# gonewest818/raytrace-clj

Hardware: NVIDIA B200
Metric: samples_per_sec (higher is better)
Workload: dtype f32

## Files before the change

### raytrace_clj_b200/csrc/rt_api.cu

```cuda
#include "../../include/raytrace_b200.h"

#include <cuda_runtime.h>
#include <dlfcn.h>
#include <math_constants.h>
#include <nccl.h>

#include <algorithm>
#include <cmath>
#include <cstdio>
#include <cstdlib>
#include <cstring>
#include <atomic>
#include <mutex>
#include <thread>
#include <string>
#include <vector>

#include "rt_bvh_build.cuh"
#include "rt_kernels.cuh"

using namespace rt;

namespace {

constexpr int kR = 4;
constexpr int kBlock = 256;
constexpr int kMinBlocks = 1;
constexpr int kTileCap = 4096;

thread_local std::string g_create_error;

struct DeviceBuffers {
    int dev = 0;
    cudaStream_t stream = nullptr;
    cudaEvent_t ev0 = nullptr, ev1 = nullptr, ev_done = nullptr;
    void* scene_blob = nullptr;
    void* scene_stage = nullptr;
    size_t scene_bytes = 0;
    DevScene sc{};
    float* d_sum = nullptr;
    float* d_mean = nullptr;
    uint8_t* d_rgb8 = nullptr;
    size_t frame_px = 0;
    unsigned long long* d_counters = nullptr;
    struct WaveLane {
        float4* queue = nullptr;
        unsigned long long* best = nullptr;
        uint2* pairs = nullptr;
        uint2* cands = nullptr;
        double* cand_t = nullptr;
        unsigned* cand_count = nullptr;
        WaveState* state = nullptr;
        LaneStatus* h_status = nullptr;
        LaneStatus* d_status = nullptr;
        cudaEvent_t ev_done = nullptr;
        cudaStream_t stream = nullptr;
        cudaStream_t stage_stream = nullptr;
        cudaEvent_t ev_culled = nullptr, ev_shaded = nullptr;
        size_t entries = 0;
        bool best_clean = false;
    } lanes[kMaxLanes];
    cudaEvent_t ev_lane_start = nullptr;
    TraceRec* d_trace = nullptr;
    struct TraceMeta { const char* kernel; int lane, iter; };
    std::vector<TraceMeta> trace_meta;
    void* scratch = nullptr;
    size_t scratch_bytes = 0;
    int sm_count = 0, clock_khz = 0;
    char name[64] = {0};
    float last_ms = 0.f;
    bool timed = false;
    float4* bvh_nodes = nullptr;
    size_t bvh_cap = 0;
    int bvh_builder = 0, bvh_depth = 0;
    long long bvh_build_ns = 0;
    void* bvh_scratch = nullptr;
    size_t bvh_scratch_bytes = 0;
    int* h_bvh_depth = nullptr;
    cudaEvent_t ev_b0 = nullptr, ev_b1 = nullptr;
    void* h_stage = nullptr;
    size_t h_stage_bytes = 0;
    cudaEvent_t ev_r0 = nullptr, ev_r1 = nullptr;
    cudaEvent_t ev_chunk[4] = {};
};

struct NcclApi {
    void* handle = nullptr;
    ncclResult_t (*CommInitAll)(ncclComm_t*, int, const int*) = nullptr;
    ncclResult_t (*CommDestroy)(ncclComm_t) = nullptr;
    ncclResult_t (*Reduce)(const void*, void*, size_t, ncclDataType_t, ncclRedOp_t, int, ncclComm_t, cudaStream_t) = nullptr;
    ncclResult_t (*GroupStart)() = nullptr;
    ncclResult_t (*GroupEnd)() = nullptr;
    const char* (*GetErrorString)(ncclResult_t) = nullptr;
    std::vector<ncclComm_t> comms;
};

}

struct Options {
    int wave_lanes = 2;
    long long wave_capacity = 1ll << 24;
    int cull_claims = 2;
    int cull_ctas_per_sm = 4;
    int cull_shape = 0;
    int light_block = 128;
    long long tail_entries = 1 << 19;
    int tail_ctas_per_sm = 0;
    int tile_records = 1024;
    int direct_spheres = 1;
    int common_origin = 1;
    int reduce = 0;
    int rows = 0;
    int tail_block = 256;
    int tail_rays = 1;
    int tail_solo = 24;
    int tail_lpp = 32;
    int mega_regcap = 0;
    int wave_depth = 2;
    int cull_tc = 1;
    int tc_tiles_per_cta = 0;
    int tc_ctas = 0;
    int bvh_build = 1;
};

struct rt_ctx {
    std::mutex mu;
    std::string err;
    std::vector<DeviceBuffers> devs;
    Options opt;
    bool has_scene = false, has_cam = false;
    int n_spheres = 0;
    int n_total = 0;
    int n_list = 0, n_cull = 0;
    int cull_cap = 0, preloaded = 0;
    int tc_tiles = 0;
    std::vector<std::vector<float>> tc_scratch_rows;
    std::vector<int> tc_row_k;
    int generic = 0;
    int accel = RT_ACCEL_BRUTE_FORCE;
    bool bvh_dirty = true;
    double win_lo = 0.0, win_hi = 0.0;
    std::vector<float> h_c0r, h_c1, h_t0t1;
    std::vector<unsigned> h_flags;
    std::vector<double> h_bs_c0, h_bs_c1, h_bs_r;
    DevCamera cam{};
    std::atomic<uint64_t> n_launches{0};
    std::mutex err_mu;
    bool profile = false;
    double stage_ms[4] = {0, 0, 0, 0};
    double reduce_ms = 0.0;
    std::vector<bool> peer_ok;
    NcclApi nccl;
};

namespace {

int fail(rt_ctx* ctx, int code, const std::string& msg) {
    if (ctx) {
        std::lock_guard<std::mutex> lk(ctx->err_mu);
        ctx->err = msg;
    } else {
        g_create_error = msg;
    }
    return code;
}

#define RT_CUDA(ctx, expr)                                                                          \
    do {                                                                                            \
        cudaError_t e__ = (expr);                                                                   \
        if (e__ != cudaSuccess)                                                                     \
            return fail(ctx, RT_ERR_CUDA, std::string(#expr) + ": " + cudaGetErrorString(e__));     \
    } while (0)

int ensure_scratch(rt_ctx* ctx, DeviceBuffers& d, size_t bytes) {
    if (d.scratch_bytes >= bytes) return RT_OK;
    if (d.scratch) cudaFree(d.scratch);
    d.scratch = nullptr;
    d.scratch_bytes = 0;
    RT_CUDA(ctx, cudaMalloc(&d.scratch, bytes));
    d.scratch_bytes = bytes;
    return RT_OK;
}

int ensure_frame(rt_ctx* ctx, DeviceBuffers& d, size_t px) {
    if (d.frame_px >= px) return RT_OK;
    if (d.d_sum) cudaFree(d.d_sum);
    if (d.d_mean) cudaFree(d.d_mean);
    if (d.d_rgb8) cudaFree(d.d_rgb8);
    d.d_sum = d.d_mean = nullptr;
    d.d_rgb8 = nullptr;
    d.frame_px = 0;
    RT_CUDA(ctx, cudaMalloc(&d.d_sum, px * 3 * sizeof(float)));
    RT_CUDA(ctx, cudaMalloc(&d.d_mean, px * 3 * sizeof(float)));
    RT_CUDA(ctx, cudaMalloc(&d.d_rgb8, px * 3));
    d.frame_px = px;
    return RT_OK;
}


void free_lane(DeviceBuffers::WaveLane& L) {
    if (L.queue) cudaFree(L.queue);
    if (L.best) cudaFree(L.best);
    if (L.pairs) cudaFree(L.pairs);
    if (L.cands) cudaFree(L.cands);
    if (L.cand_t) cudaFree(L.cand_t);
    if (L.cand_count) cudaFree(L.cand_count);
    L.queue = nullptr; L.best = nullptr; L.pairs = nullptr; L.cands = nullptr; L.cand_t = nullptr; L.cand_count = nullptr;
    L.entries = 0;
}

void free_wave(DeviceBuffers& d) {
    for (auto& L : d.lanes) {
        free_lane(L);
        if (L.state) cudaFree(L.state);
        if (L.h_status) cudaFreeHost(L.h_status);
        if (L.ev_done) cudaEventDestroy(L.ev_done);
        if (L.stream) cudaStreamDestroy(L.stream);
        if (L.stage_stream) cudaStreamDestroy(L.stage_stream);
        if (L.ev_culled) cudaEventDestroy(L.ev_culled);
        if (L.ev_shaded) cudaEventDestroy(L.ev_shaded);
        L = DeviceBuffers::WaveLane();
    }
    if (d.ev_lane_start) cudaEventDestroy(d.ev_lane_start);
    d.ev_lane_start = nullptr;
    if (d.d_trace) cudaFree(d.d_trace);
    d.d_trace = nullptr;
}

int ensure_lane(rt_ctx* ctx, DeviceBuffers& d, int lane, size_t entries) {
    DeviceBuffers::WaveLane& L = d.lanes[lane];
    if (!L.state) {
        RT_CUDA(ctx, cudaMalloc(&L.state, sizeof(WaveState)));
        RT_CUDA(ctx, cudaHostAlloc(&L.h_status, sizeof(LaneStatus), cudaHostAllocMapped));
        RT_CUDA(ctx, cudaHostGetDevicePointer((void**)&L.d_status, L.h_status, 0));
        RT_CUDA(ctx, cudaEventCreateWithFlags(&L.ev_done, cudaEventDisableTiming));
        if (lane > 0) RT_CUDA(ctx, cudaStreamCreateWithFlags(&L.stream, cudaStreamNonBlocking));
        int prio_least = 0, prio_greatest = 0;
        RT_CUDA(ctx, cudaDeviceGetStreamPriorityRange(&prio_least, &prio_greatest));
        RT_CUDA(ctx, cudaStreamCreateWithPriority(&L.stage_stream, cudaStreamNonBlocking, prio_greatest));
        RT_CUDA(ctx, cudaEventCreateWithFlags(&L.ev_culled, cudaEventDisableTiming));
        RT_CUDA(ctx, cudaEventCreateWithFlags(&L.ev_shaded, cudaEventDisableTiming));
        if (!d.ev_lane_start) RT_CUDA(ctx, cudaEventCreateWithFlags(&d.ev_lane_start, cudaEventDisableTiming));
    }
    if (L.entries >= entries) return RT_OK;
    free_lane(L);
    RT_CUDA(ctx, cudaMalloc(&L.queue, entries * 2 * 3 * sizeof(float4)));
    RT_CUDA(ctx, cudaMalloc(&L.best, entries * 2 * sizeof(unsigned long long)));
    RT_CUDA(ctx, cudaMalloc(&L.pairs, entries * kPairsPerEntry * sizeof(uint2)));
    const size_t cand_slots = entries * kPairsPerEntry + (size_t)d.sm_count * 8 * 8 * 32;
    RT_CUDA(ctx, cudaMalloc(&L.cands, cand_slots * sizeof(uint2)));
    RT_CUDA(ctx, cudaMalloc(&L.cand_t, cand_slots * sizeof(double)));
    RT_CUDA(ctx, cudaMalloc(&L.cand_count, (size_t)d.sm_count * 8 * 8 * sizeof(unsigned)));
    L.entries = entries;
    L.best_clean = false;
    return RT_OK;
}

size_t align_up(size_t x, size_t a) { return (x + a - 1) / a * a; }

float round_up_f32(double x) {
    float f = (float)x;
    if ((double)f < x) f = nextafterf(f, INFINITY);
    return f;
}

size_t mega_smem_bytes(int cull_cap) { return (size_t)cull_cap * sizeof(float4) + Culler<kR, kBlock>::LIST_BYTES; }

template <typename Kern>
int configure_kernel(rt_ctx* ctx, Kern kern, size_t smem, int* blocks_per_sm) {
    RT_CUDA(ctx, cudaFuncSetAttribute(kern, cudaFuncAttributeMaxDynamicSharedMemorySize, (int)smem));
    int b = 0;
    RT_CUDA(ctx, cudaOccupancyMaxActiveBlocksPerMultiprocessor(&b, kern, kBlock, smem));
    if (b < 1) return fail(ctx, RT_ERR_CUDA, "kernel does not fit on an SM");
    *blocks_per_sm = b;
    return RT_OK;
}

long long env_ll(const char* name, long long dflt) {
    const char* v = getenv(name);
    return (v && *v) ? atoll(v) : dflt;
}
int env_int(const char* name, int dflt) { return (int)env_ll(name, dflt); }

Options options_from_env() {
    Options o;
    o.wave_lanes = env_int("RT_WAVE_LANES", o.wave_lanes);
    o.wave_capacity = env_ll("RT_WAVE_CAPACITY", o.wave_capacity);
    o.cull_claims = env_int("RT_CULL_CLAIMS", o.cull_claims);
    o.cull_ctas_per_sm = env_int("RT_CULL_CTAS_PER_SM", o.cull_ctas_per_sm);
    const char* shape = getenv("RT_CULL_SHAPE");
    if (shape && !strcmp(shape, "128x6")) o.cull_shape = 1;
    if (shape && !strcmp(shape, "256x2")) o.cull_shape = 2;
    o.light_block = env_int("RT_LIGHT_BLOCK", o.light_block);
    o.tail_entries = env_ll("RT_TAIL_ENTRIES", o.tail_entries);
    o.tail_ctas_per_sm = env_int("RT_TAIL_CTAS_PER_SM", o.tail_ctas_per_sm);
    o.tile_records = env_int("RT_TILE_RECORDS", o.tile_records);
    o.direct_spheres = env_int("RT_DIRECT_SPHERES", o.direct_spheres);
    o.common_origin = env_int("RT_COMMON_ORIGIN", o.common_origin);
    o.reduce = env_int("RT_REDUCE", o.reduce);
    o.rows = env_int("RT_ROWS", o.rows);
    o.wave_depth = env_int("RT_WAVE_DEPTH", o.wave_depth);
    o.tail_rays = env_int("RT_TAIL_RAYS", o.tail_rays);
    o.tail_solo = env_int("RT_TAIL_SOLO", o.tail_solo);
    o.tail_lpp = env_int("RT_TAIL_LPP", o.tail_lpp);
    o.tail_block = env_int("RT_TAIL_BLOCK", o.tail_block);
    o.cull_tc = env_int("RT_CULL_TC", o.cull_tc);
    o.tc_tiles_per_cta = env_int("RT_TC_TILES_PER_CTA", o.tc_tiles_per_cta);
    o.tc_ctas = env_int("RT_TC_CTAS", o.tc_ctas);
    o.bvh_build = env_int("RT_BVH_BUILD", o.bvh_build);
    return o;
}

template <int BLOCK, int MINB>
int cull_config(rt_ctx* ctx, size_t* smem, int* bps, void (**kern)(const WaveParams)) {
    *kern = wf_cull<kR, BLOCK, MINB>;
    *smem = (ctx->preloaded ? 2 : 1) * (size_t)ctx->cull_cap * sizeof(float4) + Culler<kR, BLOCK>::LIST_BYTES;
    RT_CUDA(ctx, cudaFuncSetAttribute(*kern, cudaFuncAttributeMaxDynamicSharedMemorySize, (int)*smem));
    RT_CUDA(ctx, cudaOccupancyMaxActiveBlocksPerMultiprocessor(bps, *kern, BLOCK, *smem));
    if (*bps < 1) return fail(ctx, RT_ERR_CUDA, "cull kernel does not fit on an SM");
    return RT_OK;
}

int launch_wave(rt_ctx* ctx, DeviceBuffers& d, const RenderParams& P, unsigned long long, cudaStream_t stream) {
    const Options& opt = ctx->opt;
    void (*cull)(const WaveParams) = nullptr;
    size_t smem = 0;
    int bps = 0, cull_block = 256, rc;
    if (opt.cull_shape == 2) rc = cull_config<256, 2>(ctx, &smem, &bps, &cull);
    else if (opt.cull_shape == 1) { rc = cull_config<128, 6>(ctx, &smem, &bps, &cull); cull_block = 128; }
    else { rc = cull_config<128, 5>(ctx, &smem, &bps, &cull); cull_block = 128; }
    if (rc) return rc;
    const int cull_ctas_env = opt.cull_ctas_per_sm;
    if (cull_ctas_env > 0) bps = std::min(bps, cull_ctas_env);
    const size_t cap_env = (size_t)std::max<long long>(64, opt.wave_capacity);
    const int lanes_env = std::max(1, std::min(kMaxLanes, opt.wave_lanes));
    const int n_lanes = (ctx->profile || P.total_work < 65536) ? 1 : lanes_env;
    const size_t capacity = align_up((size_t)std::min<unsigned long long>(cap_env / n_lanes, (P.total_work + n_lanes - 1) / n_lanes), 32);

    bool done[kMaxLanes] = {};
    const unsigned tail_entries = (unsigned)std::max<long long>(0, opt.tail_entries);
    const bool gen = ctx->generic != 0;
    const bool tail4 = opt.tail_rays == 4;
    const int tail_block = (gen || tail4) ? 256 : (opt.tail_block == 32 || opt.tail_block == 64 || opt.tail_block == 128 ? opt.tail_block : 256);
    const size_t tail_smem = (size_t)ctx->cull_cap * sizeof(float4) +
                             (tail4 ? Culler<4, 256>::LIST_BYTES : (size_t)Culler<1, 256>::LIST_WORDS * tail_block * sizeof(uint32_t));
    int tail_bps = 0;
    void (*k_tail)(const WaveParams) = gen ? wf_tail<256, true, 1> : (tail4 ? wf_tail<256, false, 4> : wf_tail<256, false, 1>);
    if (tail_block == 128) k_tail = wf_tail<128, false, 1>;
    if (tail_block == 64) k_tail = wf_tail<64, false, 1>;
    if (tail_block == 32) k_tail = wf_tail<32, false, 1>;
    void (*k_refine)(const WaveParams) = gen ? wf_refine<true> : wf_refine<false>;
    void (*k_shade)(const WaveParams) = gen ? wf_shade<true> : wf_shade<false>;
    RT_CUDA(ctx, cudaFuncSetAttribute(k_tail, cudaFuncAttributeMaxDynamicSharedMemorySize, (int)tail_smem));
    RT_CUDA(ctx, cudaOccupancyMaxActiveBlocksPerMultiprocessor(&tail_bps, k_tail, tail_block, tail_smem));
    const int tail_auto = (n_lanes > 1 ? 1 : std::max(1, std::min((int)(tail_bps * tail_block / 256), 2))) * (256 / tail_block);
    const int tail_grid = d.sm_count * (opt.tail_ctas_per_sm > 0 ? opt.tail_ctas_per_sm : tail_auto);
    const bool bvh = ctx->accel == RT_ACCEL_BVH;
    void (*k_bvh)(const WaveParams) = gen ? wf_bvh<true> : wf_bvh<false>;
    const bool tail_ok = tail_bps >= 1 && tail_entries > 0 && !ctx->profile && !bvh;
    const bool use_tc = opt.cull_tc != 0 && ctx->tc_tiles > 0 && !bvh && ((ctx->n_list >= tc::MIN_LEAVES && !ctx->generic) || opt.cull_tc == 3);
    const int tc_launch_tiles = std::min(ctx->tc_tiles, (int)tc::MAX_TILES);
    const int tc_slots = tc::slots_for(tc_launch_tiles, 227 * 1024);
    const size_t tc_smem = tc::smem_bytes(tc_launch_tiles, tc_slots);
    if (use_tc) RT_CUDA(ctx, cudaFuncSetAttribute(wf_cull_tc, cudaFuncAttributeMaxDynamicSharedMemorySize, (int)tc_smem));
    const int tc_per_cta = std::max(0, opt.tc_tiles_per_cta);
    const int tc_grid = opt.tc_ctas > 0 ? std::min(opt.tc_ctas, 4 * d.sm_count) : d.sm_count;
    auto launch_tc = [&](const WaveParams& Wl, int per_cta, unsigned ctas, cudaStream_t s_) {
        WaveParams Wt = Wl;
        Wt.claims_per_warp = per_cta;
        Wt.tc_slots = tc_slots;
        for (int t0 = 0, pass = 0; t0 < ctx->tc_tiles; t0 += tc::MAX_TILES, ++pass) {
            Wt.tc_tile0 = t0;
            Wt.tc_launch_tiles = std::min((int)tc::MAX_TILES, ctx->tc_tiles - t0);
            Wt.tc_pass = pass;
            wf_cull_tc<<<ctas, tc::THREADS, tc_smem, s_>>>(Wt);
            if (pass) ctx->n_launches += 1;
        }
    };

    const int light_block = std::max(64, std::min(256, opt.light_block / 32 * 32));
    const int light_grid = d.sm_count * 8 * 256 / light_block;
    const int cull_grid = d.sm_count * bps;
    const int claims_env = std::max(0, opt.cull_claims);
    const int claims = (ctx->profile || !ctx->preloaded || n_lanes < 2 || bvh) ? 0 : claims_env;
    const int cull_warps = cull_block / 32, resident_warps = cull_grid * cull_warps;
    unsigned n_bound[kMaxLanes];
    WaveParams W[kMaxLanes];
    cudaStream_t st[kMaxLanes];
    unsigned long long first = 0;
    for (int l = 0; l < n_lanes; ++l) {
        if ((rc = ensure_lane(ctx, d, l, capacity))) return rc;
        DeviceBuffers::WaveLane& L = d.lanes[l];
        W[l] = WaveParams{};
        W[l].base = P;
        W[l].queue[0] = L.queue;
        W[l].queue[1] = L.queue + 3 * capacity;
        W[l].best_t = L.best;
        W[l].best_key = L.best + L.entries;
        W[l].pairs = L.pairs;
        W[l].cands = L.cands;
        W[l].cand_t = L.cand_t;
        W[l].cand_count = L.cand_count;
        W[l].st = L.state;
        W[l].capacity = (int)capacity;
        W[l].pair_cap = (unsigned)std::min<size_t>(capacity * kPairsPerEntry, 0xfffffff0u);
        W[l].cur = 0;
        W[l].claims_per_warp = claims;
        W[l].resident_warps = claims ? resident_warps : 0;
        W[l].tail_solo = (unsigned)std::max(0, opt.tail_solo);
        W[l].tail_lpp = opt.tail_lpp == 8 ? 8u : (opt.tail_lpp == 16 ? 16u : 32u);
        st[l] = l == 0 ? stream : L.stream;
    }
    static const char* trace_path = getenv("RT_TRACE");
    constexpr int kTraceMax = 8192;
    const bool tracing = trace_path && *trace_path;
    if (tracing) {
        if (!d.d_trace) RT_CUDA(ctx, cudaMalloc(&d.d_trace, kTraceMax * sizeof(TraceRec)));
        static const std::vector<TraceRec> init((size_t)kTraceMax, TraceRec{~0ull, 0ull});
        RT_CUDA(ctx, cudaMemcpyAsync(d.d_trace, init.data(), init.size() * sizeof(TraceRec), cudaMemcpyHostToDevice, stream));
        d.trace_meta.clear();
    }
    auto trace_slot = [&](const char* kernel, int lane, int iter) -> TraceRec* {
        if (!tracing || (int)d.trace_meta.size() >= kTraceMax) return nullptr;
        d.trace_meta.push_back({kernel, lane, iter});
        return d.d_trace + (d.trace_meta.size() - 1);
    };
    int iter_no[kMaxLanes] = {};
    static const bool debug_sync = getenv("RT_DEBUG_SYNC") && *getenv("RT_DEBUG_SYNC") == '1';
    auto dbg = [&](const char* what, int lane, int it) -> int {
        if (!debug_sync) return RT_OK;
        cudaError_t e = cudaDeviceSynchronize();
        if (e != cudaSuccess) return fail(ctx, RT_ERR_CUDA, std::string(what) + " (lane " + std::to_string(lane) + ", iteration " + std::to_string(it) + "): " + cudaGetErrorString(e));
        return RT_OK;
    };
    unsigned count0[kMaxLanes];
    unsigned long long total0 = 0;
    for (int l = 0; l < n_lanes; ++l) {
        count0[l] = (unsigned)std::min<unsigned long long>(capacity, P.total_work - total0);
        total0 += count0[l];
        n_bound[l] = count0[l];
    }
    InitParams I{};
    I.n_lanes = n_lanes;
    I.work_counter = P.work_counter;
    I.counters = P.counters;
    I.total0 = total0;
    I.total_work = P.total_work;
    for (int l = 0; l < n_lanes; ++l) {
        DeviceBuffers::WaveLane& L = d.lanes[l];
        I.st[l] = L.state;
        I.first[l] = first;
        I.count[l] = count0[l];
        first += count0[l];
        if (!L.best_clean) {
            wf_fill_best<<<d.sm_count * 4, 256, 0, stream>>>(L.best, L.best + L.entries, L.entries);
            ctx->n_launches += 1;
        }
        L.best_clean = false;
    }
    wf_init<<<1, 1, 0, stream>>>(I);
    ctx->n_launches += 1;
    RT_CUDA(ctx, cudaGetLastError());
    RT_CUDA(ctx, cudaEventRecord(d.ev_lane_start, stream));
    for (int l = 1; l < n_lanes; ++l) RT_CUDA(ctx, cudaStreamWaitEvent(st[l], d.ev_lane_start, 0));

    const int depth = std::max(1, std::min(16, opt.wave_depth));
    int enq[kMaxLanes] = {}, seen[kMaxLanes] = {};
    bool tailed[kMaxLanes] = {};
    for (int l = 0; l < n_lanes; ++l) {
        DeviceBuffers::WaveLane& L = d.lanes[l];
        memset(L.h_status, 0, sizeof(LaneStatus));
        W[l].status = L.d_status;
        if (count0[l] == 0) done[l] = true;
    }
    std::vector<cudaEvent_t> evs;
    unsigned idle_spins = 0;
    for (;;) {
        bool progressed = false, all_done = true;
        for (int l = 0; l < n_lanes; ++l) {
            if (done[l]) continue;
            all_done = false;
            DeviceBuffers::WaveLane& L = d.lanes[l];
            while (!tailed[l] && enq[l] - seen[l] < depth) {
                cudaEvent_t e[5] = {nullptr, nullptr, nullptr, nullptr, nullptr};
                if (ctx->profile)
                    for (auto& x : e) { RT_CUDA(ctx, cudaEventCreate(&x)); evs.push_back(x); }
                if (ctx->profile) cudaEventRecord(e[0], st[l]);
                W[l].iter = (unsigned)(enq[l] + 1);
                const bool tc_now = use_tc && !(enq[l] == 0 && P.common_origin && opt.cull_tc == 2);
                if (bvh) {
                    W[l].trace = trace_slot("bvh", l, iter_no[l]);
                    k_bvh<<<light_grid, 128, 0, st[l]>>>(W[l]);
                    if (ctx->profile) { cudaEventRecord(e[1], st[l]); cudaEventRecord(e[2], st[l]); cudaEventRecord(e[3], st[l]); }
                    W[l].trace = trace_slot("shade", l, iter_no[l]);
                    k_shade<<<light_grid, light_block, 0, st[l]>>>(W[l]);
                    if (ctx->profile) cudaEventRecord(e[4], st[l]);
                    ctx->n_launches -= 2;
                } else if (claims) {
                    W[l].trace = trace_slot("cull", l, iter_no[l]);
                    if (debug_sync) {
                        WaveState hs{};
                        cudaMemcpy(&hs, W[l].st, sizeof hs, cudaMemcpyDeviceToHost);
                        fprintf(stderr, "lane %d iteration %d cur %d: in flight %u fresh %u | other queue %u %u | mode %u exhausted %u npairs %u\n", l, enq[l], W[l].cur,
                                hs.cnt[W[l].cur][0], hs.cnt[W[l].cur][1], hs.cnt[W[l].cur ^ 1][0], hs.cnt[W[l].cur ^ 1][1], hs.mode, hs.exhausted, hs.npairs);
                    }
                    if (tc_now) {
                        const unsigned tiles = (n_bound[l] + tc::TILE_M - 1) / tc::TILE_M;
                        const unsigned ctas = tc_per_cta ? (tiles + (unsigned)tc_per_cta - 1u) / (unsigned)tc_per_cta : (unsigned)tc_grid;
                        launch_tc(W[l], tc_per_cta, std::max(1u, ctas), st[l]);
// ... 11 lines not shown
                    W[l].trace = trace_slot("tiebreak", l, iter_no[l]);
                    wf_tiebreak<<<light_grid, light_block, 0, L.stage_stream>>>(W[l]);
                    if ((rc = dbg("wf_tiebreak", l, enq[l]))) return rc;
                    W[l].trace = trace_slot("shade", l, iter_no[l]);
                    k_shade<<<light_grid, light_block, 0, L.stage_stream>>>(W[l]);
                    if ((rc = dbg("wf_shade", l, enq[l]))) return rc;
                    RT_CUDA(ctx, cudaEventRecord(L.ev_shaded, L.stage_stream));
                    RT_CUDA(ctx, cudaStreamWaitEvent(st[l], L.ev_shaded, 0));
                } else {
                    W[l].trace = trace_slot("cull", l, iter_no[l]);
                    if (tc_now) {
                        launch_tc(W[l], 0, (unsigned)tc_grid, st[l]);
                    } else {
                        cull<<<cull_grid, cull_block, smem, st[l]>>>(W[l]);
                    }
                    if (ctx->profile) cudaEventRecord(e[1], st[l]);
                    W[l].trace = trace_slot("refine", l, iter_no[l]);
                    k_refine<<<light_grid, light_block, 0, st[l]>>>(W[l]);
                    if (ctx->profile) cudaEventRecord(e[2], st[l]);
                    W[l].trace = trace_slot("tiebreak", l, iter_no[l]);
                    wf_tiebreak<<<light_grid, light_block, 0, st[l]>>>(W[l]);
                    if (ctx->profile) cudaEventRecord(e[3], st[l]);
                    W[l].trace = trace_slot("shade", l, iter_no[l]);
                    k_shade<<<light_grid, light_block, 0, st[l]>>>(W[l]);
                    if (ctx->profile) cudaEventRecord(e[4], st[l]);
                }
                RT_CUDA(ctx, cudaGetLastError());
                W[l].cur ^= 1;
                ++iter_no[l];
                ctx->n_launches += 4;
                ++enq[l];
                progressed = true;
            }
        }
        if (all_done) break;
        for (int l = 0; l < n_lanes; ++l) {
            if (done[l]) continue;
            DeviceBuffers::WaveLane& L = d.lanes[l];
            const volatile LaneStatus* hs = L.h_status;
            const unsigned seq = hs->seq;
            if ((int)seq == seen[l] && hs->mode != MODE_DONE) continue;
            std::atomic_thread_fence(std::memory_order_acquire);
            const unsigned n_next = hs->n_next, n_fresh = hs->n_fresh, exhausted = hs->exhausted, mode = hs->mode;
            if (hs->seq != seq) continue;
            seen[l] = (int)seq;
            progressed = true;
            if (exhausted) n_bound[l] = std::min(n_bound[l], n_next);
            if (mode == MODE_DONE) { done[l] = true; continue; }
            if (tail_ok && !tailed[l] && exhausted && n_fresh == 0 && n_next <= tail_entries) {
                W[l].iter = (unsigned)(enq[l] + 1);
                W[l].trace = trace_slot("tail", l, iter_no[l]);
                k_tail<<<tail_grid, tail_block, tail_smem, st[l]>>>(W[l]);
                if ((rc = dbg("wf_tail", l, enq[l]))) return rc;
                RT_CUDA(ctx, cudaGetLastError());
                ctx->n_launches += 1;
                tailed[l] = true;
            }
        }
        if (!progressed) {
            if (++idle_spins > 200) {
                if (cudaSuccess != cudaPeekAtLastError()) RT_CUDA(ctx, cudaGetLastError());
                if (idle_spins > 20000 && (idle_spins % 1000) == 0) {
                    for (int l = 0; l < n_lanes; ++l)
                        if (!done[l] && cudaStreamQuery(st[l]) == cudaSuccess && d.lanes[l].h_status->seq == (unsigned)seen[l] &&
                            enq[l] > seen[l])
                            return fail(ctx, RT_ERR_CUDA, "wavefront lane finished its queue without reporting status");
                }
                std::this_thread::yield();
            }
        } else {
            idle_spins = 0;
        }
    }
    for (int l = 1; l < n_lanes; ++l) {
        RT_CUDA(ctx, cudaEventRecord(d.lanes[l].ev_done, st[l]));
        RT_CUDA(ctx, cudaStreamWaitEvent(stream, d.lanes[l].ev_done, 0));
    }
    for (int l = 0; l < n_lanes; ++l) d.lanes[l].best_clean = true;
    if (ctx->profile) {
        RT_CUDA(ctx, cudaStreamSynchronize(stream));
        for (size_t i = 0; i + 4 < evs.size(); i += 5)
            for (int sgi = 0; sgi < 4; ++sgi) {
                float ms = 0.f;
                if (cudaEventElapsedTime(&ms, evs[i + sgi], evs[i + sgi + 1]) == cudaSuccess) ctx->stage_ms[sgi] += ms;
            }
        for (auto x : evs) cudaEventDestroy(x);
    }
    return RT_OK;
}

int launch_params(rt_ctx* ctx, DeviceBuffers& d, RenderParams& P, int variant, cudaStream_t stream);

int launch_render(rt_ctx* ctx, DeviceBuffers& d, int nx, int ny, int sample_begin, int sample_count, int row_offset,
                  int row_stride, int max_depth, uint64_t seed, int variant, float* d_sum, cudaStream_t stream) {
    RenderParams P{};
    P.sc = d.sc;
    P.cam = ctx->cam;
    P.nx = nx;
    P.ny = ny;
    P.sample_begin = sample_begin;
    P.sample_count = sample_count;
    P.row_offset = row_offset;
    P.row_stride = row_stride;
    P.rows_in_shard = (ny - row_offset + row_stride - 1) / row_stride;
    P.max_depth = max_depth;
    P.key = make_uint2((uint32_t)seed, (uint32_t)(seed >> 32));
    P.sum = d_sum;
    P.counters = d.d_counters;
// ... 873 lines not shown
    if (accel != RT_ACCEL_BRUTE_FORCE && accel != RT_ACCEL_BVH) return fail(ctx, RT_ERR_ARG, "unknown accelerator");
    ctx->accel = accel;
    if (accel == RT_ACCEL_BVH && ctx->has_scene) return ensure_bvh(ctx);
    return RT_OK;
}

int rt_get_bvh(rt_ctx* ctx, int device_index, float* out_nodes, int64_t cap_nodes, int64_t info[4]) {
    if (!ctx) return RT_ERR_ARG;
    std::lock_guard<std::mutex> lk(ctx->mu);
    if (int rc = check_ready(ctx)) return rc;
    if (device_index < 0 || device_index >= (int)ctx->devs.size()) return fail(ctx, RT_ERR_ARG, "device_index out of range");
    if (int rc = ensure_bvh(ctx)) return rc;
    DeviceBuffers& d = ctx->devs[(size_t)device_index];
    const int64_t n_nodes = d.sc.bvh_nodes;
    if (info) {
        info[0] = n_nodes;
        info[1] = d.bvh_depth;
        info[2] = d.bvh_builder;
        info[3] = d.bvh_build_ns;
    }
    if (out_nodes) {
        if (cap_nodes < n_nodes) return fail(ctx, RT_ERR_ARG, "cap_nodes is below the node count (info[0])");
        RT_CUDA(ctx, cudaSetDevice(d.dev));
        RT_CUDA(ctx, cudaMemcpy(out_nodes, d.bvh_nodes, (size_t)n_nodes * 4 * sizeof(float4), cudaMemcpyDeviceToHost));
        cudaSetDevice(ctx->devs[0].dev);
    }
    return RT_OK;
}

int rt_set_option(rt_ctx* ctx, const char* name, int64_t value) {
    if (!ctx) return RT_ERR_ARG;
    std::lock_guard<std::mutex> lk(ctx->mu);
    if (!name) return fail(ctx, RT_ERR_ARG, "option name is null");
    Options& o = ctx->opt;
    const std::string k(name);
    if (k == "wave_lanes") o.wave_lanes = (int)value;
    else if (k == "wave_capacity") o.wave_capacity = value;
    else if (k == "cull_claims") o.cull_claims = (int)value;
    else if (k == "cull_ctas_per_sm") o.cull_ctas_per_sm = (int)value;
    else if (k == "cull_shape") o.cull_shape = (int)value;
    else if (k == "light_block") o.light_block = (int)value;
    else if (k == "tail_entries") o.tail_entries = value;
    else if (k == "tail_ctas_per_sm") o.tail_ctas_per_sm = (int)value;
    else if (k == "tile_records") o.tile_records = (int)value;
    else if (k == "direct_spheres") o.direct_spheres = (int)value;
    else if (k == "common_origin") o.common_origin = (int)value;
    else if (k == "reduce") o.reduce = (int)value;
    else if (k == "rows") o.rows = (int)value;
    else if (k == "wave_depth") o.wave_depth = (int)value;
    else if (k == "mega_regcap") o.mega_regcap = (int)value;
    else if (k == "tail_rays") o.tail_rays = (int)value;
    else if (k == "tail_solo") o.tail_solo = (int)value;
    else if (k == "tail_lpp") o.tail_lpp = (int)value;
    else if (k == "tail_block") o.tail_block = (int)value;
    else if (k == "cull_tc") o.cull_tc = (int)value;
    else if (k == "tc_tiles_per_cta") o.tc_tiles_per_cta = (int)value;
    else if (k == "tc_ctas") o.tc_ctas = (int)value;
    else if (k == "bvh_build") o.bvh_build = (int)value;
    else return fail(ctx, RT_ERR_ARG, "unknown option: " + k);
    return RT_OK;
}

int rt_set_camera(rt_ctx* ctx, int cam_type, const float cam[24]) {
    if (!ctx) return RT_ERR_ARG;
    std::lock_guard<std::mutex> lk(ctx->mu);
    if (!cam) return fail(ctx, RT_ERR_ARG, "cam is null");
    if (cam_type != RT_CAM_PINHOLE && cam_type != RT_CAM_THIN_LENS) return fail(ctx, RT_ERR_UNSUPPORTED, "unknown camera type");
    DevCamera& c = ctx->cam;
    c.type = cam_type;
    auto g = [&](int k) { return make_float3(cam[3 * k], cam[3 * k + 1], cam[3 * k + 2]); };
    c.origin = g(0); c.lleft = g(1); c.horiz = g(2); c.vert = g(3); c.u = g(4); c.v = g(5); c.w = g(6);
    c.lens_radius = cam[21] / 2.0f;
    c.t0 = cam[22];
    c.t1 = cam[23];
    ctx->has_cam = true;
    return RT_OK;
}

int rt_render_accumulate_device(rt_ctx* ctx, int nx, int ny, int sample_begin, int sample_count, int row_offset,
                                int row_stride, int max_depth, uint64_t seed, int variant, float* d_sum, void* stream,
                                int sync) {
    int rc = check_ready(ctx);
    if (rc) return rc;
    std::lock_guard<std::mutex> lk(ctx->mu);
    if ((rc = check_camera_times(ctx))) return rc;
    if (nx <= 0 || ny <= 0 || sample_count < 0 || sample_begin < 0 || max_depth < 0 || !d_sum || row_stride < 1 ||
        row_offset < 0 || row_offset >= row_stride)
        return fail(ctx, RT_ERR_ARG, "bad render arguments");
    if ((long long)nx * ny > 0x7fffffffLL / 3) return fail(ctx, RT_ERR_ARG, "image too large");
    DeviceBuffers& d = ctx->devs[0];
    RT_CUDA(ctx, cudaSetDevice(d.dev));
    cudaStream_t st = (cudaStream_t)stream;
    RT_CUDA(ctx, cudaEventRecord(d.ev0, st));
    rc = launch_render(ctx, d, nx, ny, sample_begin, sample_count, row_offset, row_stride, max_depth, seed, variant, d_sum, st);
    if (rc) return rc;
    RT_CUDA(ctx, cudaEventRecord(d.ev1, st));
    d.timed = true;
    if (sync) RT_CUDA(ctx, cudaStreamSynchronize(st));
    return RT_OK;
}

int rt_resolve_device(rt_ctx* ctx, int nx, int ny, int nsamples_total, const float* d_sum, uint8_t* d_rgb8, void* stream,
                      int sync) {
    if (!ctx) return RT_ERR_ARG;
    std::lock_guard<std::mutex> lk(ctx->mu);
    if (nx <= 0 || ny <= 0 || nsamples_total <= 0 || !d_sum || !d_rgb8) return fail(ctx, RT_ERR_ARG, "bad resolve arguments");
// ... 584 lines not shown
```

### raytrace_clj_b200/csrc/rt_kernels.cuh

```cuda
#pragma once

#include "rt_device.cuh"

namespace rt {

#define RT_FOR_R _Pragma("unroll") for (int r = 0; r < R; ++r)

struct PathBounce {
    float o[3];
    float time;
    float d[3];
    int hit_id;
    double t;
};

struct RenderParams {
    DevScene sc;
    DevCamera cam;
    int nx, ny;
    int sample_begin, sample_count;
    int row_offset, row_stride, rows_in_shard;
    int max_depth;
    uint2 key;
    float* sum;
// ... 302 lines not shown
struct LaneStatus {
    unsigned n_next;
    unsigned n_fresh;
    unsigned exhausted;
    unsigned mode;
    unsigned seq;
    unsigned pad[3];
};
__device__ __forceinline__ unsigned wf_entry(unsigned i, unsigned n_g, unsigned n_p, unsigned capacity) {
    return i < n_g ? i : capacity - n_p + (i - n_g);
}

struct TraceRec {
    unsigned long long t_start, t_end;
};
__device__ __forceinline__ unsigned long long global_timer_ns() {
    unsigned long long t;
    asm volatile("mov.u64 %0, %globaltimer;" : "=l"(t));
    return t;
}
struct TraceScope {
    TraceRec* rec;
    __device__ __forceinline__ explicit TraceScope(TraceRec* r) : rec(r) {
        if (rec && threadIdx.x == 0) atomicMin(&rec->t_start, global_timer_ns());
    }
    __device__ __forceinline__ ~TraceScope() {
        if (rec && threadIdx.x == 0) atomicMax(&rec->t_end, global_timer_ns());
    }
};

struct WaveParams {
    RenderParams base;
    float4* queue[2];
    unsigned long long* best_t;
    unsigned long long* best_key;
    uint2* pairs;
    uint2* cands;
    double* cand_t;
    unsigned* cand_count;
    WaveState* st;
    int capacity;
    unsigned pair_cap;
    int cur;
    int claims_per_warp;
    int resident_warps;
    volatile LaneStatus* status;
    unsigned iter;
    TraceRec* trace;
    int tc_slots;
    int tc_tile0, tc_launch_tiles;
    int tc_pass;
    unsigned tail_solo;
    unsigned tail_lpp;
};
__device__ __forceinline__ void publish_status(const WaveParams& W, unsigned n_next, unsigned n_fresh, unsigned exhausted, unsigned mode,
                                               unsigned seq) {
    if (!W.status) return;
    W.status->n_next = n_next;
    W.status->n_fresh = n_fresh;
    W.status->exhausted = exhausted;
    W.status->mode = mode;
    __threadfence_system();
    W.status->seq = seq;
}

constexpr unsigned long long BEST_T_INIT = 0x7ff0000000000000ull;
constexpr unsigned long long BEST_KEY_MISS = ~0ull;
constexpr unsigned long long BEST_KEY_OVERFLOW = 0ull;
constexpr unsigned PAIR_NULL = 0xffffffffu;

__device__ __forceinline__ unsigned warp_claim(unsigned* counter, bool pred, unsigned lane) {
    unsigned m = __ballot_sync(0xffffffffu, pred);
    unsigned base = 0;
    if (m) {
        int leader = __ffs(m) - 1;
        if ((int)lane == leader) base = atomicAdd(counter, (unsigned)__popc(m));
        base = __shfl_sync(0xffffffffu, base, leader);
    }
    return base + __popc(m & ((1u << lane) - 1u));
}

__device__ __forceinline__ void make_path(const RenderParams& P, unsigned long long w, float4& a, float4& b, float4& c) {
    const unsigned pshard = (unsigned)P.nx * (unsigned)P.rows_in_shard;
    unsigned s_local, q;
    if (P.total_work <= 0xffffffffull) {
        s_local = (unsigned)w / pshard;
        q = (unsigned)w - s_local * pshard;
    } else {
        s_local = (unsigned)(w / pshard);
        q = (unsigned)(w - (unsigned long long)s_local * pshard);
    }
    int row_local = (int)(q / (unsigned)P.nx);
    int i = (int)(q - (unsigned)row_local * (unsigned)P.nx);
    int j = P.row_offset + row_local * P.row_stride;
    uint32_t pix = (uint32_t)j * (uint32_t)P.nx + (uint32_t)i;
    uint32_t smp = (uint32_t)(P.sample_begin + (int)s_local);
    uint32_t slot = pix;
    if (P.path_pixel) {
        pix = (uint32_t)__ldg(&P.path_pixel[w]);
        smp = (uint32_t)__ldg(&P.path_sample[w]);
        j = (int)(pix / (uint32_t)P.nx);
        i = (int)(pix - (uint32_t)j * (uint32_t)P.nx);
        slot = (uint32_t)w;
    }
    float3 o, d;
    float tmv;
// ... 635 lines not shown
                                                      bounce);
                    const unsigned long long tb = (unsigned long long)__double_as_longlong(t);
                    const unsigned long long kk = (((unsigned long long)__ldg(&P.sc.tie_hi[s])) << 32) | (unsigned)s;
                    if (t < CUDART_INF && (tb < bt || (tb == bt && kk < bkey))) { bt = tb; bkey = kk; }
                }
            }
        }
        for (unsigned dlt = lpp >> 1; dlt; dlt >>= 1) {
            const unsigned long long ot = __shfl_xor_sync(0xffffffffu, bt, (int)dlt), ok = __shfl_xor_sync(0xffffffffu, bkey, (int)dlt);
            if (ot < bt || (ot == bt && ok < bkey)) { bt = ot; bkey = ok; }
        }
        if (active) {
            const bool hit = bkey != BEST_KEY_MISS;
            const int k = (int)(unsigned)bkey;
            const double td = __longlong_as_double((long long)bt);
            if (P.path_pixel && sub == 0u) path_log_ray(P, slot, (int)bounce - 1, a, b, hit ? k : -1, hit ? td : CUDART_INF);
            int reason = TERM_MISS;
            bool cont = false;
            if (hit) {
                float3 o = f3(a.x, a.y, a.z), d = f3(b.x, b.y, b.z);
                float3 att, em;
                float tmv = a.w;
                ScatterRng rng{P.key, pix, smp, bounce, nullptr, nullptr};
                reason = TERM_NONE;
                cont = shade_hit<GEN>(P.sc, scp, k, (float)td, o, d, tmv, depth > 0, rng, att, em, reason);
                if (sub == 0u && (em.x != 0.f || em.y != 0.f || em.z != 0.f)) {
                    float* dst = P.sum + (size_t)slot * 3;
                    atomicAdd(dst + 0, c.x * em.x);
                    atomicAdd(dst + 1, c.y * em.y);
                    atomicAdd(dst + 2, c.z * em.z);
                }
                if (cont) {
                    a = make_float4(o.x, o.y, o.z, tmv);
                    b = make_float4(d.x, d.y, d.z, b.w);
                    c = make_float4(c.x * att.x, c.y * att.y, c.z * att.z, __uint_as_float((smp << 8) | (uint32_t)(depth - 1)));
                }
            }
            if (!cont) {
                if (sub == 0u) {
                    atomicAdd(&s_ctr[reason == TERM_MISS ? DC_TERM_MISS : reason == TERM_LIGHT ? DC_TERM_LIGHT
                                     : reason == TERM_ABSORB ? DC_TERM_ABSORB : DC_TERM_DEPTH], 1u);
                    if (P.path_pixel) path_log_end(P, slot, (int)bounce, reason);
                }
                active = false;
            }
        }
    }
    if (n_rays) atomicAdd(&s_ctr[DC_RAYS], n_rays);
    if (n_cand) atomicAdd(&s_ctr[DC_CANDIDATES], n_cand);
    if (n_direct) atomicAdd(&s_ctr[DC_DIRECT], n_direct);
}

constexpr int kPairsPerEntry = 8;
template <int BLOCK, bool GEN, int TR>
__global__ void __launch_bounds__(BLOCK, GEN ? 1 : 2) wf_tail(const __grid_constant__ WaveParams W) {
    const RenderParams& P = W.base;
    extern __shared__ float4 smem_f4[];
    float4* s_cull = smem_f4;
    uint32_t* s_list = reinterpret_cast<uint32_t*>(smem_f4 + P.cull_cap);
    __shared__ unsigned s_ctr[DC_COUNT];
    __shared__ WaveState s_st;
    if (W.st->mode == MODE_DONE) return;
    TraceScope trace(W.trace);
    int cur = W.cur;
    const unsigned n_all = W.st->cnt[cur][0];
    const unsigned K = ((n_all + gridDim.x - 1) / gridDim.x + 31u) / 32u * 32u;
    const unsigned first = blockIdx.x * K;
    if (first < n_all) {
        if (threadIdx.x < DC_COUNT) s_ctr[threadIdx.x] = 0;
        if (threadIdx.x == 0) {
            s_st.cnt[cur][0] = min(K, n_all - first);
            s_st.cnt[cur ^ 1][0] = 0;
            s_st.cnt[0][1] = s_st.cnt[1][1] = 0;
            s_st.gen_base[0] = s_st.gen_base[1] = 0ull;
            s_st.batch = 0;
            s_st.npairs = 0;
            s_st.exhausted = 1;
            s_st.done = 0;
            s_st.mode = MODE_RUN;
            s_st.pad = 0;
        }
        const unsigned warps = BLOCK / 32;
        WaveParams L = W;
        L.queue[0] = W.queue[0] + 3 * (size_t)first;
        L.queue[1] = W.queue[1] + 3 * (size_t)first;
        L.best_t = W.best_t + first;
        L.best_key = W.best_key + first;
        L.pairs = W.pairs + (size_t)first * kPairsPerEntry;
        L.pair_cap = min(K, (unsigned)W.capacity - first) * kPairsPerEntry;
        const size_t cand_slice = (size_t)wf_cand_region(L, warps) * warps;
        L.cands = W.cands + (size_t)blockIdx.x * cand_slice;
        L.cand_t = W.cand_t + (size_t)blockIdx.x * cand_slice;
        L.cand_count = W.cand_count + blockIdx.x * warps;
        L.st = &s_st;
        L.status = nullptr;
        L.capacity = (int)K;
        L.claims_per_warp = 0;
        L.resident_warps = 0;
        if (P.preloaded) preload_scene(P.sc, s_cull, BLOCK);
        const Scope solo{0u, 1u};
        for (;;) {
            __syncthreads();
            const unsigned n = *(volatile unsigned*)&s_st.cnt[cur][0];
#ifdef RT_TAIL_DIAG
            const bool diag = (blockIdx.x == 0 || blockIdx.x == gridDim.x / 2) && threadIdx.x == 0;
            unsigned long long dt0 = global_timer_ns();
#endif
            if (n <= W.tail_solo) {
                if (n) wf_solo_paths<GEN>(L, &W.base.sc, cur ? L.queue[1] : L.queue[0], n, &s_st.done, s_cull, s_ctr);
#ifdef RT_TAIL_DIAG
                __syncthreads();
                if (diag) printf("tail cta %u solo n %u: %llu ns\n", blockIdx.x, n, global_timer_ns() - dt0);
#endif
                break;
            }
            wf_cull_body<TR, BLOCK>(L, solo, cur, n, 0u, 0ull, s_cull, nullptr, s_list);
            __syncthreads();
#ifdef RT_TAIL_DIAG
            unsigned long long dt1 = global_timer_ns();
            const unsigned np_ = s_st.npairs;
#endif
            wf_refine_body<GEN>(L, &W.base.sc, solo, cur);
            __syncthreads();
#ifdef RT_TAIL_DIAG
            unsigned long long dt2 = global_timer_ns();
#endif
            wf_tiebreak_body(L, solo);
            __syncthreads();
#ifdef RT_TAIL_DIAG
            unsigned long long dt3 = global_timer_ns();
#endif
            wf_shade_body<GEN>(L, &W.base.sc, solo, cur, s_ctr);
#ifdef RT_TAIL_DIAG
            __syncthreads();
            if (diag) printf("tail cta %u n %u pairs %u: cull %llu refine %llu tie %llu shade %llu ns\n", blockIdx.x, n, np_, dt1 - dt0, dt2 - dt1, dt3 - dt2, global_timer_ns() - dt3);
#endif
            cur ^= 1;
        }
        __syncthreads();
        if (threadIdx.x < DC_COUNT && s_ctr[threadIdx.x]) atomicAdd(&P.counters[threadIdx.x], (unsigned long long)s_ctr[threadIdx.x]);
    }
    if (threadIdx.x == 0) {
        __threadfence();
        if (atomicAdd(&W.st->done, 1u) == gridDim.x - 1) {
            W.st->done = 0;
            W.st->cnt[0][0] = W.st->cnt[0][1] = W.st->cnt[1][0] = W.st->cnt[1][1] = 0;
            W.st->mode = MODE_DONE;
            __threadfence();
            publish_status(W, 0u, 0u, 1u, MODE_DONE, W.iter);
        }
    }
}


struct MegaShade {
    float4 o_t;
    float4 d_c;
    float4 att_r;
    float4 em;
};
template <bool GEN>
__device__ __noinline__ MegaShade mega_shade_one(const DevScene* scp, int k, float t, float ox, float oy, float oz, float dx, float dy,
                                                 float dz, float time, int allow_scatter, uint2 key, uint32_t pix, uint32_t smp,
                                                 uint32_t bounce) {
    float3 o = f3(ox, oy, oz), d = f3(dx, dy, dz), att, em;
    int reason = TERM_NONE;
    ScatterRng rng{key, pix, smp, bounce, nullptr, nullptr};
    const bool cont = shade_hit<GEN>(*scp, scp, k, t, o, d, time, allow_scatter != 0, rng, att, em, reason);
    MegaShade m;
    m.o_t = make_float4(o.x, o.y, o.z, time);
    m.d_c = make_float4(d.x, d.y, d.z, cont ? 1.f : 0.f);
    m.att_r = make_float4(att.x, att.y, att.z, (float)reason);
    m.em = make_float4(em.x, em.y, em.z, 0.f);
    return m;
}

template <int R, int BLOCK, int MINB, bool GEN>
__global__ void __launch_bounds__(BLOCK, MINB) mega_kernel(const __grid_constant__ RenderParams P) {
    extern __shared__ float4 smem_f4[];
    float4* s_cull = smem_f4;
    uint32_t* s_list = reinterpret_cast<uint32_t*>(smem_f4 + P.cull_cap);
    __shared__ unsigned s_ctr[DC_COUNT];
    if (threadIdx.x < DC_COUNT) s_ctr[threadIdx.x] = 0;
    if (P.preloaded) preload_scene(P.sc, s_cull, BLOCK);
    __syncthreads();

    Culler<R, BLOCK> K;
    RefineSink<R, BLOCK, GEN> I;
    I.tmin = 0.001;
    I.tmax = (double)FLT_MAX;
    I.ncand = 0;
    I.sc = &P.sc;
    I.has_ctx = true;
    I.key = P.key;

    float ar[R], ag[R], ab[R];
    uint32_t slot[R];
    uint32_t (&pix)[R] = I.pix, (&smp)[R] = I.smp;
    int depth[R];
    bool alive[R];
    RT_FOR_R { alive[r] = false; I.ox[r] = I.oy[r] = I.oz[r] = I.tm[r] = 0.f; I.dx[r] = 1.f; I.dy[r] = I.dz[r] = 0.f; pix[r] = smp[r] = slot[r] = 0u; I.bounce[r] = 0u; }
    unsigned n_rays = 0, n_samples = 0, n_direct = 0;
    const unsigned lane = threadIdx.x & 31u;
    const unsigned pshard = (unsigned)P.nx * (unsigned)P.rows_in_shard;
// ... 303 lines not shown
```

Baseline: 1.621 billion.

## Hand thin tail workloads to register-resident kernel with split-sphere culling

Adds a wf_thin kernel that runs after wf_tail. When a CTA's remaining ray count drops to tail_thin or below, wf_tail records the count and queue index per block and exits instead of looping through the cull/refine/tiebreak/shade stages. wf_thin keeps each ray in registers, splits culling of the sphere list across warps with per-part best-hit reduction in shared memory, then shades and compacts survivors with ballot. The aim is to cut per-bounce stage and barrier overhead when few rays are left, at the cost of an extra launch per lane, a per-lane slice buffer and its memset, and more shared memory.

```diff
diff --git a/raytrace_clj_b200/csrc/rt_api.cu b/raytrace_clj_b200/csrc/rt_api.cu
--- a/raytrace_clj_b200/csrc/rt_api.cu
+++ b/raytrace_clj_b200/csrc/rt_api.cu
@@ -57,6 +57,8 @@
         cudaStream_t stream = nullptr;
         cudaStream_t stage_stream = nullptr;
         cudaEvent_t ev_culled = nullptr, ev_shaded = nullptr;
+        uint2* thin_slice = nullptr;
+        int thin_slots = 0;
         size_t entries = 0;
         bool best_clean = false;
     } lanes[kMaxLanes];
@@ -115,6 +117,7 @@
     int tail_rays = 1;
     int tail_solo = 24;
     int tail_lpp = 32;
+    int tail_thin = 256;
     int mega_regcap = 0;
     int wave_depth = 2;
     int cull_tc = 1;
@@ -219,6 +222,7 @@
         if (L.stage_stream) cudaStreamDestroy(L.stage_stream);
         if (L.ev_culled) cudaEventDestroy(L.ev_culled);
         if (L.ev_shaded) cudaEventDestroy(L.ev_shaded);
+        if (L.thin_slice) cudaFree(L.thin_slice);
         L = DeviceBuffers::WaveLane();
     }
     if (d.ev_lane_start) cudaEventDestroy(d.ev_lane_start);
@@ -303,6 +307,7 @@
     o.tail_rays = env_int("RT_TAIL_RAYS", o.tail_rays);
     o.tail_solo = env_int("RT_TAIL_SOLO", o.tail_solo);
     o.tail_lpp = env_int("RT_TAIL_LPP", o.tail_lpp);
+    o.tail_thin = env_int("RT_TAIL_THIN", o.tail_thin);
     o.tail_block = env_int("RT_TAIL_BLOCK", o.tail_block);
     o.cull_tc = env_int("RT_CULL_TC", o.cull_tc);
     o.tc_tiles_per_cta = env_int("RT_TC_TILES_PER_CTA", o.tc_tiles_per_cta);
@@ -358,6 +363,14 @@
     const bool bvh = ctx->accel == RT_ACCEL_BVH;
     void (*k_bvh)(const WaveParams) = gen ? wf_bvh<true> : wf_bvh<false>;
     const bool tail_ok = tail_bps >= 1 && tail_entries > 0 && !ctx->profile && !bvh;
+    const bool thin_ok = tail_ok && opt.tail_thin > 0 && ctx->preloaded;
+    void (*k_thin)(const WaveParams) = gen ? wf_thin<256, true> : wf_thin<256, false>;
+    if (tail_block == 128) k_thin = wf_thin<128, false>;
+    if (tail_block == 64) k_thin = wf_thin<64, false>;
+    if (tail_block == 32) k_thin = wf_thin<32, false>;
+    const size_t thin_smem = (size_t)ctx->cull_cap * sizeof(float4) + (size_t)Culler<1, 256>::LIST_WORDS * tail_block * sizeof(uint32_t) +
+                             (size_t)tail_block * (3 * sizeof(float4) + sizeof(ulonglong2));
+    if (thin_ok) RT_CUDA(ctx, cudaFuncSetAttribute(k_thin, cudaFuncAttributeMaxDynamicSharedMemorySize, (int)thin_smem));
     const bool use_tc = opt.cull_tc != 0 && ctx->tc_tiles > 0 && !bvh && ((ctx->n_list >= tc::MIN_LEAVES && !ctx->generic) || opt.cull_tc == 3);
     const int tc_launch_tiles = std::min(ctx->tc_tiles, (int)tc::MAX_TILES);
     const int tc_slots = tc::slots_for(tc_launch_tiles, 227 * 1024);
@@ -391,6 +404,14 @@
     for (int l = 0; l < n_lanes; ++l) {
         if ((rc = ensure_lane(ctx, d, l, capacity))) return rc;
         DeviceBuffers::WaveLane& L = d.lanes[l];
+        if (thin_ok && L.thin_slots < tail_grid) {
+            if (L.thin_slice) cudaFree(L.thin_slice);
+            L.thin_slice = nullptr;
+            L.thin_slots = 0;
+            RT_CUDA(ctx, cudaMalloc(&L.thin_slice, (size_t)tail_grid * sizeof(uint2)));
+            RT_CUDA(ctx, cudaMemset(L.thin_slice, 0, (size_t)tail_grid * sizeof(uint2)));
+            L.thin_slots = tail_grid;
+        }
         W[l] = WaveParams{};
         W[l].base = P;
         W[l].queue[0] = L.queue;
@@ -409,6 +430,8 @@
         W[l].resident_warps = claims ? resident_warps : 0;
         W[l].tail_solo = (unsigned)std::max(0, opt.tail_solo);
         W[l].tail_lpp = opt.tail_lpp == 8 ? 8u : (opt.tail_lpp == 16 ? 16u : 32u);
+        W[l].tail_thin = thin_ok ? (unsigned)std::min(opt.tail_thin, tail_block) : 0u;
+        W[l].thin_slice = L.thin_slice;
         st[l] = l == 0 ? stream : L.stream;
     }
     static const char* trace_path = getenv("RT_TRACE");
@@ -455,6 +478,7 @@
         if (!L.best_clean) {
             wf_fill_best<<<d.sm_count * 4, 256, 0, stream>>>(L.best, L.best + L.entries, L.entries);
             ctx->n_launches += 1;
+            if (L.thin_slice) RT_CUDA(ctx, cudaMemsetAsync(L.thin_slice, 0, (size_t)L.thin_slots * sizeof(uint2), stream));
         }
         L.best_clean = false;
     }
@@ -572,8 +596,14 @@
                 W[l].trace = trace_slot("tail", l, iter_no[l]);
                 k_tail<<<tail_grid, tail_block, tail_smem, st[l]>>>(W[l]);
                 if ((rc = dbg("wf_tail", l, enq[l]))) return rc;
+                ctx->n_launches += 1;
+                if (thin_ok) {
+                    W[l].trace = trace_slot("thin", l, iter_no[l]);
+                    k_thin<<<tail_grid, tail_block, thin_smem, st[l]>>>(W[l]);
+                    if ((rc = dbg("wf_thin", l, enq[l]))) return rc;
+                    ctx->n_launches += 1;
+                }
                 RT_CUDA(ctx, cudaGetLastError());
-                ctx->n_launches += 1;
                 tailed[l] = true;
             }
         }
@@ -1553,6 +1583,7 @@
     else if (k == "tail_rays") o.tail_rays = (int)value;
     else if (k == "tail_solo") o.tail_solo = (int)value;
     else if (k == "tail_lpp") o.tail_lpp = (int)value;
+    else if (k == "tail_thin") o.tail_thin = (int)value;
     else if (k == "tail_block") o.tail_block = (int)value;
     else if (k == "cull_tc") o.cull_tc = (int)value;
     else if (k == "tc_tiles_per_cta") o.tc_tiles_per_cta = (int)value;
diff --git a/raytrace_clj_b200/csrc/rt_kernels.cuh b/raytrace_clj_b200/csrc/rt_kernels.cuh
--- a/raytrace_clj_b200/csrc/rt_kernels.cuh
+++ b/raytrace_clj_b200/csrc/rt_kernels.cuh
@@ -378,6 +378,8 @@
     int tc_pass;
     unsigned tail_solo;
     unsigned tail_lpp;
+    unsigned tail_thin;
+    uint2* thin_slice;
 };
 __device__ __forceinline__ void publish_status(const WaveParams& W, unsigned n_next, unsigned n_fresh, unsigned exhausted, unsigned mode,
                                                unsigned seq) {
@@ -1119,6 +1121,16 @@
 }
 
 constexpr int kPairsPerEntry = 8;
+__device__ __forceinline__ void wf_drain_lane(const WaveParams& W) {
+    __threadfence();
+    if (atomicAdd(&W.st->done, 1u) == gridDim.x - 1) {
+        W.st->done = 0;
+        W.st->cnt[0][0] = W.st->cnt[0][1] = W.st->cnt[1][0] = W.st->cnt[1][1] = 0;
+        W.st->mode = MODE_DONE;
+        __threadfence();
+        publish_status(W, 0u, 0u, 1u, MODE_DONE, W.iter);
+    }
+}
 template <int BLOCK, bool GEN, int TR>
 __global__ void __launch_bounds__(BLOCK, GEN ? 1 : 2) wf_tail(const __grid_constant__ WaveParams W) {
     const RenderParams& P = W.base;
@@ -1181,6 +1193,10 @@
 #endif
                 break;
             }
+            if (n <= W.tail_thin) {
+                if (threadIdx.x == 0) W.thin_slice[blockIdx.x] = make_uint2(n, (unsigned)cur);
+                break;
+            }
             wf_cull_body<TR, BLOCK>(L, solo, cur, n, 0u, 0ull, s_cull, nullptr, s_list);
             __syncthreads();
 #ifdef RT_TAIL_DIAG
@@ -1207,16 +1223,191 @@
         __syncthreads();
         if (threadIdx.x < DC_COUNT && s_ctr[threadIdx.x]) atomicAdd(&P.counters[threadIdx.x], (unsigned long long)s_ctr[threadIdx.x]);
     }
-    if (threadIdx.x == 0) {
-        __threadfence();
-        if (atomicAdd(&W.st->done, 1u) == gridDim.x - 1) {
-            W.st->done = 0;
-            W.st->cnt[0][0] = W.st->cnt[0][1] = W.st->cnt[1][0] = W.st->cnt[1][1] = 0;
-            W.st->mode = MODE_DONE;
-            __threadfence();
-            publish_status(W, 0u, 0u, 1u, MODE_DONE, W.iter);
-        }
-    }
+    if (W.tail_thin == 0u && threadIdx.x == 0) wf_drain_lane(W);
+}
+
+template <int BLOCK, bool GEN>
+struct ThinSink {
+    float ox, oy, oz, dx, dy, dz, tm;
+    uint32_t pix, smp, bounce;
+    uint2 key;
+    const DevScene* sc;
+    unsigned long long bt, bkey;
+    unsigned ncand;
+
+    __device__ __forceinline__ void flush(const uint32_t* list, unsigned long long nz, int count, int kbase) {
+        SurvivorIter<1, BLOCK> it;
+        it.begin(nz, count);
+        int r, k;
+        while (it.next(list, r, k)) {
+            k += kbase;
+            ++ncand;
+            const double t = refine_leaf<GEN>(sc, k, ox, oy, oz, dx, dy, dz, tm, 0.001, (double)FLT_MAX, true, key, pix, smp, bounce);
+            const unsigned long long tb = (unsigned long long)__double_as_longlong(t);
+            const unsigned long long kk = (((unsigned long long)__ldg(&sc->tie_hi[k])) << 32) | (unsigned)k;
+            if (t < CUDART_INF && (tb < bt || (tb == bt && kk < bkey))) { bt = tb; bkey = kk; }
+        }
+    }
+};
+
+template <int BLOCK, bool GEN>
+__global__ void __launch_bounds__(BLOCK, GEN ? 1 : 2) wf_thin(const __grid_constant__ WaveParams W) {
+    constexpr int WARPS = BLOCK / 32;
+    const RenderParams& P = W.base;
+    const DevScene* scp = &W.base.sc;
+    extern __shared__ float4 smem_f4[];
+    float4* s_cull = smem_f4;
+    uint32_t* s_list = reinterpret_cast<uint32_t*>(smem_f4 + P.cull_cap);
+    float4* s_ray = reinterpret_cast<float4*>(s_list + Culler<1, BLOCK>::LIST_WORDS * BLOCK);
+    ulonglong2* s_part = reinterpret_cast<ulonglong2*>(s_ray + 3 * BLOCK);
+    __shared__ unsigned s_ctr[DC_COUNT];
+    __shared__ unsigned s_warp[WARPS];
+    if (W.st->mode == MODE_DONE) return;
+    TraceScope trace(W.trace);
+    const unsigned n_all = W.st->cnt[W.cur][0];
+    const unsigned K = ((n_all + gridDim.x - 1) / gridDim.x + 31u) / 32u * 32u;
+    const unsigned first = blockIdx.x * K;
+    const uint2 h = first < n_all ? W.thin_slice[blockIdx.x] : make_uint2(0u, 0u);
+    unsigned n = h.x;
+    if (n) {
+        const unsigned lane = threadIdx.x & 31u, warp = threadIdx.x >> 5;
+        const float4* qc = (h.y ? W.queue[1] : W.queue[0]) + 3 * (size_t)first;
+        bool live = threadIdx.x < n;
+        float4 a = make_float4(0.f, 0.f, 0.f, 0.f), b = a, c = a;
+        uint32_t slot = 0u, pix = 0u;
+        if (live) {
+            a = qc[3 * threadIdx.x]; b = qc[3 * threadIdx.x + 1]; c = qc[3 * threadIdx.x + 2];
+            slot = __float_as_uint(b.w);
+            pix = rng_pixel(P, slot);
+        }
+        unsigned rank = threadIdx.x, n_rays = 0, n_cand = 0, n_direct = 0;
+        if (threadIdx.x < DC_COUNT) s_ctr[threadIdx.x] = 0;
+        preload_scene(P.sc, s_cull, BLOCK);
+        if (threadIdx.x == 0) W.thin_slice[blockIdx.x] = make_uint2(0u, 0u);
+        while (n) {
+#ifdef RT_TAIL_DIAG
+            const bool diag = (blockIdx.x == 0 || blockIdx.x == gridDim.x / 2) && threadIdx.x == 0;
+            const unsigned long long dt0 = global_timer_ns();
+#endif
+            const uint32_t sd = __float_as_uint(c.w), smp = sd >> 8;
+            const int depth = (int)(sd & 255u);
+            const uint32_t bounce = (uint32_t)(P.max_depth - depth + 1);
+            n_rays += n;
+            if (live) {
+                s_ray[rank] = a;
+                s_ray[BLOCK + rank] = b;
+                if (GEN) s_ray[2 * BLOCK + rank] = make_float4(__uint_as_float(pix), __uint_as_float(smp), __uint_as_float(bounce), 0.f);
+            }
+            __syncthreads();
+            const unsigned b1 = (n + 31u) / 32u;
+            unsigned parts = 1;
+            while (b1 * parts * 2u <= (unsigned)WARPS) parts *= 2;
+            for (unsigned item = warp; item < b1 * parts; item += WARPS) {
+                const unsigned batch = item / parts, part = item - batch * parts, v = batch * 32u + lane;
+                Culler<1, BLOCK> Kc;
+                ThinSink<BLOCK, GEN> sink;
+                sink.sc = scp;
+                sink.key = P.key;
+                sink.bt = BEST_T_INIT;
+                sink.bkey = BEST_KEY_MISS;
+                sink.ncand = 0;
+                if (v < n) {
+                    const float4 ra = s_ray[v], rb = s_ray[BLOCK + v];
+                    sink.ox = ra.x; sink.oy = ra.y; sink.oz = ra.z; sink.tm = ra.w;
+                    sink.dx = rb.x; sink.dy = rb.y; sink.dz = rb.z;
+                    if (GEN) {
+                        const float4 rc = s_ray[2 * BLOCK + v];
+                        sink.pix = __float_as_uint(rc.x); sink.smp = __float_as_uint(rc.y); sink.bounce = __float_as_uint(rc.z);
+                    } else {
+                        sink.pix = sink.smp = sink.bounce = 0u;
+                    }
+                    Kc.set_ray(0, ra.x, ra.y, ra.z, rb.x, rb.y, rb.z);
+                } else {
+                    sink.ox = sink.oy = sink.oz = sink.dx = sink.dy = sink.dz = sink.tm = 0.f;
+                    sink.pix = sink.smp = sink.bounce = 0u;
+                    Kc.kill(0);
+                }
+                Kc.run_slice(P.sc, s_cull, s_list, sink, (int)part, (int)parts);
+                n_cand += sink.ncand;
+                s_part[part * b1 * 32u + v] = make_ulonglong2(sink.bt, sink.bkey);
+            }
+            __syncthreads();
+#ifdef RT_TAIL_DIAG
+            const unsigned long long dt1 = global_timer_ns();
+#endif
+            bool cont = false;
+            if (live) {
+                unsigned long long tb = BEST_T_INIT, key = BEST_KEY_MISS;
+                for (unsigned p = 0; p < parts; ++p) {
+                    const ulonglong2 q = s_part[p * b1 * 32u + rank];
+                    if (q.x < tb || (q.x == tb && q.y < key)) { tb = q.x; key = q.y; }
+                }
+                int k = (int)(unsigned)key;
+                double td = __longlong_as_double((long long)tb);
+                for (int kd = P.sc.n_list; kd < P.sc.n; ++kd) {
+                    ++n_direct;
+                    const double t = refine_leaf<GEN>(scp, kd, a.x, a.y, a.z, b.x, b.y, b.z, a.w, 0.001, (double)FLT_MAX, true, P.key, pix,
+                                                      smp, bounce);
+                    const unsigned long long kk = (((unsigned long long)__ldg(&P.sc.tie_hi[kd])) << 32) | (unsigned)kd;
+                    if (t < td || (t < CUDART_INF && t == td && kk < key)) {
+                        td = t;
+                        key = kk;
+                        k = kd;
+                    }
+                }
+                const bool hit = key != BEST_KEY_MISS;
+                if (P.path_pixel) path_log_ray(P, slot, (int)bounce - 1, a, b, hit ? k : -1, hit ? td : CUDART_INF);
+                if (!hit) {
+                    atomicAdd(&s_ctr[DC_TERM_MISS], 1u);
+                    if (P.path_pixel) path_log_end(P, slot, (int)bounce, TERM_MISS);
+                } else {
+                    float3 o = f3(a.x, a.y, a.z), d = f3(b.x, b.y, b.z);
+                    float3 att, em;
+                    int reason = TERM_NONE;
+                    float tmv = a.w;
+                    ScatterRng rng{P.key, pix, smp, bounce, nullptr, nullptr};
+                    cont = shade_hit<GEN>(P.sc, scp, k, (float)td, o, d, tmv, depth > 0, rng, att, em, reason);
+                    if (em.x != 0.f || em.y != 0.f || em.z != 0.f) {
+                        float* dst = P.sum + (size_t)slot * 3;
+                        atomicAdd(dst + 0, c.x * em.x);
+                        atomicAdd(dst + 1, c.y * em.y);
+                        atomicAdd(dst + 2, c.z * em.z);
+                    }
+                    if (cont) {
+                        a = make_float4(o.x, o.y, o.z, tmv);
+                        b = make_float4(d.x, d.y, d.z, b.w);
+                        c = make_float4(c.x * att.x, c.y * att.y, c.z * att.z, __uint_as_float((smp << 8) | (uint32_t)(depth - 1)));
+                    } else {
+                        atomicAdd(&s_ctr[reason == TERM_LIGHT ? DC_TERM_LIGHT
+                                         : reason == TERM_ABSORB ? DC_TERM_ABSORB : DC_TERM_DEPTH], 1u);
+                        if (P.path_pixel) path_log_end(P, slot, (int)bounce, reason);
+                    }
+                }
+            }
+            const unsigned mc = __ballot_sync(0xffffffffu, cont);
+            if (lane == 0) s_warp[warp] = (unsigned)__popc(mc);
+            __syncthreads();
+            unsigned base = 0, total = 0;
+#pragma unroll
+            for (int w = 0; w < WARPS; ++w) {
+                const unsigned cw = s_warp[w];
+                if (w < (int)warp) base += cw;
+                total += cw;
+            }
+            rank = base + __popc(mc & ((1u << lane) - 1u));
+            live = cont;
+#ifdef RT_TAIL_DIAG
+            if (diag) printf("thin cta %u n %u: cull+refine %llu shade %llu ns\n", blockIdx.x, n, dt1 - dt0, global_timer_ns() - dt1);
+#endif
+            n = total;
+        }
+        if (n_cand) atomicAdd(&s_ctr[DC_CANDIDATES], n_cand);
+        if (n_direct) atomicAdd(&s_ctr[DC_DIRECT], n_direct);
+        if (threadIdx.x == 0) s_ctr[DC_RAYS] += n_rays;
+        __syncthreads();
+        if (threadIdx.x < DC_COUNT && s_ctr[threadIdx.x]) atomicAdd(&P.counters[threadIdx.x], (unsigned long long)s_ctr[threadIdx.x]);
+    }
+    if (threadIdx.x == 0) wf_drain_lane(W);
 }
 
 
```

Result: no change. 1.636 billion (median of 6 runs) (+1.0%).
